# seorim0/DNN-based-Speech-Enhancement-in-the-frequency-domain

Measured on AMD Instinct MI355X. Metric: train utts/sec (3s@16kHz) DCCRN, higher is better.
Workload: dtype bf16; 1 GPU; DCCRN mask C, SI-SNR, fwd+bwd+Adam, B=32/GPU x 3s@16kHz clips (BASELINE configs[1]); global_batch=32, parallelism=dp1, bn=per-rank statistics, collective=none

## Files before the change

dnn-based-speech-enhancement-in-the-frequency-domain_amd/csrc/dev_common.h:

```cpp
#pragma once
#include <hip/hip_runtime.h>
#include "sefd_desc.h"

namespace sefd {

typedef __attribute__((ext_vector_type(4))) float f32x4;
typedef __attribute__((ext_vector_type(16))) float f32x16;
typedef __attribute__((ext_vector_type(8))) __bf16 bf16x8;

struct bf16_t { uint16_t v; };

struct ArenaBases { char* p[A_COUNT]; int* status; int* dstatus; };
__device__ __forceinline__ void set_status(int* host_word, int* dev_word) {
  if (host_word) __hip_atomic_store(host_word, 1, __ATOMIC_RELAXED, __HIP_MEMORY_SCOPE_SYSTEM);
  if (dev_word) __hip_atomic_store(dev_word, 1, __ATOMIC_RELAXED, __HIP_MEMORY_SCOPE_AGENT);
}

__host__ __device__ __forceinline__ char* rp(const ArenaBases& ab, const Ptr& q) { return ab.p[q.arena] + q.off; }

__device__ __forceinline__ uint32_t pack_bf16x2(float lo, float hi) {
  uint32_t r;
  asm("v_cvt_pk_bf16_f32 %0, %1, %2" : "=v"(r) : "v"(lo), "v"(hi));
  return r;
}
// ... 92 lines not shown
__device__ __forceinline__ float tanhf_(float x) { return 1.f - 2.f * __builtin_amdgcn_rcpf(__expf(2.f * x) + 1.f); }

__device__ __forceinline__ uint32_t mix32(uint32_t a, uint32_t b, uint32_t c) {
  uint32_t x = a * 0x9E3779B1u ^ (b + 0x7F4A7C15u) * 0x85EBCA77u ^ (c + 0x632BE5ABu) * 0xC2B2AE3Du;
  x ^= x >> 16; x *= 0x7FEB352Du; x ^= x >> 15; x *= 0x846CA68Bu; x ^= x >> 16;
  return x;
}
__device__ __forceinline__ float drop_scale(uint32_t seed0, uint32_t seed1, int layer, float keep, int64_t i) {
  if (keep >= 1.f) return 1.f;
  const uint32_t r = mix32(seed0 + (uint32_t)layer * 0x51ED27u, seed1 ^ (uint32_t)(i >> 32), (uint32_t)i);
  return ((r >> 8) * (1.f / 16777216.f)) < keep ? 1.f / keep : 0.f;
}

struct BnbCol { float mean, invstd, gamma, beta; };
__device__ __forceinline__ BnbCol bnb_col(const RunGemm& d, const ArenaBases& ab, int n) {
  BnbCol c{0.f, 0.f, 0.f, 0.f};
  if (n < d.N) {
    const float* mi = reinterpret_cast<const float*>(rp(ab, d.bnb_mi));
    c.mean = mi[n]; c.invstd = mi[d.N + n];
    c.gamma = reinterpret_cast<const float*>(rp(ab, d.bnb_gamma))[n];
    c.beta = reinterpret_cast<const float*>(rp(ab, d.bnb_beta))[n];
  }
  return c;
}
__device__ __forceinline__ void bnb_accum(const BnbCol& c, float slope, float dz, float yf, float& s0, float& s1, float& s2) {
  const float xh = (yf - c.mean) * c.invstd;
  const float bn = c.gamma * xh + c.beta;
  const float dbn = bn > 0.f ? dz : slope * dz;
  s0 += dbn;
  s1 += dbn * xh;
  s2 += bn > 0.f ? 0.f : bn * dz;
}

struct StreamKey {
  int dev; hipStream_t st;
  bool operator==(const StreamKey& o) const { return dev == o.dev && st == o.st; }
};
struct StreamKeyHash { size_t operator()(const StreamKey& k) const { return (size_t)(uintptr_t)k.st * 31u + (size_t)k.dev; } };
inline StreamKey stream_key(hipStream_t st) { int dev = 0; (void)hipGetDevice(&dev); return StreamKey{dev, st}; }

void launch_rungemm(const RunGemm& d, const ArenaBases& ab, hipStream_t st);
void launch_wgrad(const RunGemm& d, const ArenaBases& ab, hipStream_t st);
bool launch_cgemm256(const RunGemm& d, const ArenaBases& ab, hipStream_t st);
bool launch_enc0_fwd(const RunGemm& d, const ArenaBases& ab, hipStream_t st);
bool launch_enc0_wgrad(const RunGemm& d, const ArenaBases& ab, hipStream_t st);
bool launch_rundirect(const RunGemm& d, const ArenaBases& ab, hipStream_t st);
bool rundirect_takes(const RunGemm& d);
bool launch_rungemm_persist(const RunGemm& d, const ArenaBases& ab, hipStream_t st);
int rungemm_persist_grid(const RunGemm& d);
bool launch_thin_mask(const RunGemm& d, const ArenaBases& ab, hipStream_t st);
int thin_mask_grid(const RunGemm& d);
bool launch_thin_stage(const RunGemm& d, const ArenaBases& ab, hipStream_t st);
int thin_stage_grid(const RunGemm& d);
enum RunFamily : int { kFamNone = 0, kFamEnc0 = 1, kFamCgemm256 = 2, kFamDirect = 3, kFamTiled = 4, kFamPersist = 5, kFamThinMask = 6, kFamThinStage = 7 };
int rungemm_family(const RunGemm& d);
enum WgradFamily : int { kWgFamNone = 0, kWgFamEnc0 = 1, kWgFamEnc0Fused = 2, kWgFamRank = 3, kWgFamWide256 = 4, kWgFamWide256Ones = 5, kWgFamWide128 = 6,
                         kWgFamDma128 = 7, kWgFamDma64 = 8, kWgFamDma32 = 9, kWgFamBf16_128 = 10, kWgFamBf16_64 = 11, kWgFamF32 = 12, kWgFamThin = 13 };
int wgrad_family(const RunGemm& d);
bool launch_thin_wgrad(const RunGemm& d, const ArenaBases& ab, hipStream_t st);
bool thin_wgrad_takes(const RunGemm& d);
void launch_misc(const Op& op, const ArenaBases& ab, hipStream_t st);
void launch_stft_fft(const StftFft& d, const ArenaBases& ab, hipStream_t st);
void launch_istft_fft(const IstftFft& d, const ArenaBases& ab, hipStream_t st);
void launch_ifft_ola(const IfftOla& d, const ArenaBases& ab, hipStream_t st);
void launch_specconv(const SpecConv& d, const ArenaBases& ab, hipStream_t st);
void launch_ola_fold(const Ola& d, const ArenaBases& ab, hipStream_t st);
void launch_specout_adj(const SpecOut& d, const ArenaBases& ab, hipStream_t st);
void launch_nchw_cl(const NchwCl& d, const ArenaBases& ab, hipStream_t st);
void launch_fsn(const Op& op, const ArenaBases& ab, hipStream_t st);
void launch_bn(const Op& op, const ArenaBases& ab, hipStream_t st);
void launch_cbn(const Op& op, const ArenaBases& ab, hipStream_t st);
void launch_lstm_bf16(const LstmRec& d, const ArenaBases& ab, hipStream_t st, bool fwd);
inline int lstm_rev_groups(const LstmRec& d) { return d.rev_mask & ((1 << (d.G < 4 ? d.G : 4)) - 1); }
void launch_lstm_cluster(const LstmRec& d, const ArenaBases& ab, hipStream_t st, bool fwd);
void launch_lstm_rows(const LstmRec& d, const ArenaBases& ab, hipStream_t st, bool fwd);
bool launch_lstm_rows_pair(const LstmRec& d0, const LstmRec& d1, const ArenaBases& ab, hipStream_t st);

}
```

dnn-based-speech-enhancement-in-the-frequency-domain_amd/csrc/rungemm.hip:

```cpp
#include <hip/hip_runtime.h>
#include <cstdlib>
#include "sefd_desc.h"
#include "tuning.h"
#include "dev_common.h"

namespace sefd {

template <typename TA>
struct RowInfo {
  int64_t base0, base1;
  int32_t u, fo;
  bool valid;
};

template <typename TA>
__device__ __forceinline__ uint4 load_a_chunk(const RunGemm& d, const TA* x0, const TA* x1, const Seg& sg,
                                              int64_t base0, int64_t base1, int u, int fo, bool rvalid, int j0) {
  constexpr int VEC = 16 / sizeof(TA);
  uint4 z = make_uint4(0, 0, 0, 0);
  if (!rvalid) return z;
  if (sg.src < 0) {
    if (j0 == 0) {
      if (sizeof(TA) == 4) z.x = 0x3f800000u; else z.x = 0x3f80u;
    }
// ... 1106 lines not shown
}

static bool launch_wgrad_rank(const RunGemm& d, const ArenaBases& ab, hipStream_t st) {
  if (!(d.flags & kRunRank) || !wgrad_rank_form(d)) return false;
  const dim3 grid((unsigned)d.nsplit);
  if (d.N <= 2) hipLaunchKernelGGL((wgrad_rank_kernel<2>), grid, dim3(256), 0, st, d, ab);
  else hipLaunchKernelGGL((wgrad_rank_kernel<4>), grid, dim3(256), 0, st, d, ab);
  return true;
}

template <typename TA, int BN>
static void launch_rungemm_dma(const RunGemm& d, const ArenaBases& ab, hipStream_t st, int grid) {
  if (d.flags & kRunBnBwd) { hipLaunchKernelGGL((rungemm_kernel<TA, BN, true, 2, kBM, 4, false, true>), dim3(grid), dim3(256), 0, st, d, ab); return; }
  hipLaunchKernelGGL((rungemm_kernel<TA, BN, true, 2>), dim3(grid), dim3(256), 0, st, d, ab);
}

template <typename TA>
static void launch_rungemm_t(const RunGemm& d, const ArenaBases& ab, hipStream_t st) {
  const int bn = bn_of(d.N);
  const int nm = (d.M + kBM - 1) / kBM;
  const int grid = nm * (d.Npad / bn);
  if constexpr (sizeof(TA) == 2) {
    if (launch_rungemm_persist(d, ab, st)) return;
  }
  if (d.flags & kRunAligned) {
    if (bn == 128) launch_rungemm_dma<TA, 128>(d, ab, st, grid);
    else if (bn == 64) launch_rungemm_dma<TA, 64>(d, ab, st, grid);
    else launch_rungemm_dma<TA, 32>(d, ab, st, grid);
    return;
  }
  if (d.flags & kRunBnBwd) {
    if (bn == 128) hipLaunchKernelGGL((rungemm_kernel<TA, 128, false, 2, kBM, 4, false, true>), dim3(grid), dim3(256), 0, st, d, ab);
    else if (bn == 64) hipLaunchKernelGGL((rungemm_kernel<TA, 64, false, 2, kBM, 4, false, true>), dim3(grid), dim3(256), 0, st, d, ab);
    else hipLaunchKernelGGL((rungemm_kernel<TA, 32, false, 2, kBM, 4, false, true>), dim3(grid), dim3(256), 0, st, d, ab);
    return;
  }
  if (bn == 128) hipLaunchKernelGGL((rungemm_kernel<TA, 128, false>), dim3(grid), dim3(256), 0, st, d, ab);
  else if (bn == 64) hipLaunchKernelGGL((rungemm_kernel<TA, 64, false>), dim3(grid), dim3(256), 0, st, d, ab);
  else hipLaunchKernelGGL((rungemm_kernel<TA, 32, false>), dim3(grid), dim3(256), 0, st, d, ab);
}

__global__ void refuse_launch_kernel(int* host_word, int* dev_word) { set_status(host_word, dev_word); }

static void refuse_launch(const ArenaBases& ab, hipStream_t st) {
  hipLaunchKernelGGL(refuse_launch_kernel, dim3(1), dim3(1), 0, st, ab.status, ab.dstatus);
}

void launch_rungemm(const RunGemm& d, const ArenaBases& ab, hipStream_t st) {
  if (launch_enc0_fwd(d, ab, st)) return;
  if (d.flags & (kRunEnc0 | kRunDyFromBn)) { refuse_launch(ab, st); return; }
  if (launch_cgemm256(d, ab, st)) return;
  if (launch_thin_mask(d, ab, st)) return;
  if (launch_thin_stage(d, ab, st)) return;
  if (launch_rundirect(d, ab, st)) return;
  if (d.xdt == DT_BF16) launch_rungemm_t<bf16_t>(d, ab, st);
  else launch_rungemm_t<float>(d, ab, st);
}

int rungemm_family(const RunGemm& d) {
  if ((d.flags & kRunEnc0) && enc0_accepts(d, false)) return kFamEnc0;
  if (d.flags & (kRunEnc0 | kRunDyFromBn)) return kFamNone;
  if (d.flags & kRunWTile32) return kFamCgemm256;
  if (thin_mask_grid(d) > 0) return kFamThinMask;
  if (thin_stage_grid(d) > 0) return kFamThinStage;
  if (rundirect_takes(d)) return kFamDirect;
  if (d.xdt == DT_BF16 && rungemm_persist_grid(d) > 0) return kFamPersist;
  return kFamTiled;
}

static void launch_wgrad_wide(const RunGemm& d, const ArenaBases& ab, hipStream_t st) {
  if (d.flags & kRunOnesMfma) {
    dim3 grid1(((d.Npad + 255) / 256) * ((d.ldw - 64 + 255) / 256) * d.nsplit);
    hipLaunchKernelGGL((wgrad_bf16_dma_kernel<256, 4, 256, 512, true, true>), grid1, dim3(512), 0, st, d, ab);
    return;
  }
  dim3 grid(((d.Npad + 255) / 256) * ((d.ldw + 255) / 256) * d.nsplit);
  hipLaunchKernelGGL((wgrad_bf16_dma_kernel<256, 4, 256, 512, true>), grid, dim3(512), 0, st, d, ab);
}

static void launch_wgrad_wide128(const RunGemm& d, const ArenaBases& ab, hipStream_t st) {
  dim3 grid(((d.Npad + 127) / 128) * ((d.ldw + 511) / 512) * d.nsplit);
  hipLaunchKernelGGL((wgrad_bf16_dma_kernel<128, 2, 512, 512>), grid, dim3(512), 0, st, d, ab);
}

template <int TN>
static void launch_wgrad_dma(const RunGemm& d, const ArenaBases& ab, hipStream_t st) {
  dim3 grid(((d.Npad + TN - 1) / TN) * ((d.ldw + kWgTK - 1) / kWgTK) * d.nsplit);
  hipLaunchKernelGGL((wgrad_bf16_dma_kernel<TN, 3>), grid, dim3(256), 0, st, d, ab);
}

void launch_wgrad(const RunGemm& d0, const ArenaBases& ab, hipStream_t st) {
  if (launch_enc0_wgrad(d0, ab, st)) return;
  if (d0.flags & (kRunEnc0 | kRunDyFromBn)) { refuse_launch(ab, st); return; }
  if (launch_wgrad_rank(d0, ab, st)) return;
  RunGemm d = d0;
#ifdef SEFD_TUNING
  if (tune_int("WG_DBG", 0) & 8) d.flags |= 1 << 30;
#endif
  if (d.xdt == DT_BF16 && (d.flags & kRunAligned)) {
    if (d.flags & kRunWgWide) { if (d.Npad % 256 == 0) launch_wgrad_wide(d, ab, st); else launch_wgrad_wide128(d, ab, st); return; }
    if (launch_thin_wgrad(d0, ab, st)) return;
    switch (wgrad_tn(d.xdt, d.N, d.Npad)) {
      case 128: launch_wgrad_dma<128>(d, ab, st); break;
      case 64: launch_wgrad_dma<64>(d, ab, st); break;
      default: launch_wgrad_dma<32>(d, ab, st); break;
    }
    return;
  }
  if (d.xdt == DT_BF16) {
    if (d.Npad >= 128) {
      dim3 grid(((d.Npad + 127) / 128) * ((d.ldw + kWgTK - 1) / kWgTK) * d.nsplit);
      hipLaunchKernelGGL((wgrad_bf16_kernel<128>), grid, dim3(256), 0, st, d, ab);
    } else {
      dim3 grid(((d.Npad + 63) / 64) * ((d.ldw + kWgTK - 1) / kWgTK) * d.nsplit);
      hipLaunchKernelGGL((wgrad_bf16_kernel<64>), grid, dim3(256), 0, st, d, ab);
    }
    return;
// ... 24 lines not shown
```

dnn-based-speech-enhancement-in-the-frequency-domain_amd/csrc/thin_stage.hip:

```cpp
#include <hip/hip_runtime.h>
#include <cstdlib>
#include "sefd_desc.h"
#include "tuning.h"
#include "dev_common.h"

namespace sefd {

namespace {

constexpr int kStageFo = 64;
constexpr int64_t kThinStageMinRows = 262144;

__device__ __forceinline__ void settle(f32x4& a, f32x4& b) { asm volatile("s_nop 7\n\ts_nop 7" : "+v"(a), "+v"(b)); }
__device__ __forceinline__ void settle(f32x4& a, f32x4& b, f32x4& c, f32x4& e) { asm volatile("s_nop 7\n\ts_nop 7" : "+v"(a), "+v"(b), "+v"(c), "+v"(e)); }

template <int CTRL>
__device__ __forceinline__ float dpp_f(float x) {
  return __builtin_bit_cast(float, __builtin_amdgcn_update_dpp(0, __builtin_bit_cast(int, x), CTRL, 0xF, 0xF, true));
}
__device__ __forceinline__ void chain32(float a, float b, float& t1, float& t2) {
  constexpr int SHR1 = 0x111, SHR5 = 0x115, SHL11 = 0x10B, SHL4 = 0x104;
  float s = 0.f + a, r = __builtin_fmaf(a, a, 0.f);
#pragma unroll
  for (int k = 0; k < 3; ++k) { s = dpp_f<SHR1>(s) + a; r = __builtin_fmaf(a, a, dpp_f<SHR1>(r)); }
  s = dpp_f<SHR5>(s) + a; r = __builtin_fmaf(a, a, dpp_f<SHR5>(r));
#pragma unroll
  for (int k = 0; k < 3; ++k) { s = dpp_f<SHR1>(s) + a; r = __builtin_fmaf(a, a, dpp_f<SHR1>(r)); }
  s = dpp_f<SHL11>(s) + b; r = __builtin_fmaf(b, b, dpp_f<SHL11>(r));
#pragma unroll
  for (int k = 0; k < 3; ++k) { s = dpp_f<SHR1>(s) + b; r = __builtin_fmaf(b, b, dpp_f<SHR1>(r)); }
  s = dpp_f<SHR5>(s) + b; r = __builtin_fmaf(b, b, dpp_f<SHR5>(r));
#pragma unroll
  for (int k = 0; k < 3; ++k) { s = dpp_f<SHR1>(s) + b; r = __builtin_fmaf(b, b, dpp_f<SHR1>(r)); }
  t1 = s + dpp_f<SHL4>(s);
  t2 = r + dpp_f<SHL4>(r);
}
__device__ __forceinline__ void chain32(const f32x4& a, const f32x4& b, f32x4& t1, f32x4& t2) {
#pragma unroll
  for (int e = 0; e < 4; ++e) { float x, y; chain32(a[e], b[e], x, y); t1[e] = x; t2[e] = y; }
}

template <int C, int NSRC>
struct StageGeom {
  static constexpr int CH = NSRC * C / 8;
  static constexpr int PB = CH * 16;
  static constexpr int SLOT = (kStageFo + 2) * PB;
  static constexpr int CPT = C / 8;
  static constexpr int HS = C / 32;
  static constexpr int NSEG = 2 * NSRC;
  static constexpr int KS = NSEG * 3 * HS;
  static constexpr int NIT = kStageFo * CH / 256;
  static constexpr int RPL = PB >= 256 ? 1 : 256 / PB;
  static constexpr int NT = C / 16;
  static constexpr int NPG = 4 / NT;
  static constexpr int NB = kStageFo / 16 / NPG;
  static constexpr int RED = NPG > 1 ? 2 * 4 * 2 * 4 * 16 : 0;
  static_assert((C == 64 || C == 32) && (NSRC == 1 || NSRC == 2) && NIT >= 1 && NB % 2 == 0 && NT * NPG == 4 && (NPG == 1 || NB == 2), "instantiated forms");
  __host__ __device__ static constexpr int swz(int pos) { return (pos / RPL) & (CH - 1); }
};

}

template <int C, int NSRC>
// ... 118 lines not shown
        float* prow = part + (int64_t)(g >> 1) * 2 * d.Npad + 16 * ct + 4 * q;
        if constexpr (G::NPG == 1) {
          if (fr == 0) { s1 = f32x4{0.f, 0.f, 0.f, 0.f}; s2 = s1; }
#pragma unroll
          for (int j = 0; j < NB / 2; ++j) {
            f32x4 t1, t2;
            chain32(acc[2 * j], acc[2 * j + 1], t1, t2);
            s1 += t1; s2 += t2;
          }
          if (rowend && li == 11) {
            *reinterpret_cast<f32x4*>(prow) = s1;
            *reinterpret_cast<f32x4*>(prow + d.Npad) = s2;
          }
        } else {
          f32x4* red = reinterpret_cast<f32x4*>(smem + 3 * SLOT);
          f32x4 t1, t2;
          chain32(acc[0], acc[1], t1, t2);
          if (li == 11) { red[((fr * 4 + wid) * 2 + 0) * 4 + q] = t1; red[((fr * 4 + wid) * 2 + 1) * 4 + q] = t2; }
          if (rowend) {
            lds_barrier();
            if (pg == 0 && li == 11) {
              f32x4 a1 = {0.f, 0.f, 0.f, 0.f}, a2 = a1;
              for (int f = 0; f <= fr; ++f)
#pragma unroll
                for (int h = 0; h < G::NPG; ++h) { a1 += red[((f * 4 + ct + h * NT) * 2 + 0) * 4 + q]; a2 += red[((f * 4 + ct + h * NT) * 2 + 1) * 4 + q]; }
              *reinterpret_cast<f32x4*>(prow) = a1;
              *reinterpret_cast<f32x4*>(prow + d.Npad) = a2;
            }
          }
        }
      }

      uint16_t* yrow = y + (int64_t)cb * d.y_bstride + (int64_t)cu * d.y_tstride + d.y_off + 16 * ct + (odd ? 4 * (q - 1) : 4 * q);
#pragma unroll
      for (int j = 0; j < NB / 2; ++j) {
        const f32x4 &A = acc[2 * j], &B = acc[2 * j + 1];
        const uint32_t X0 = pack_bf16x2(A[0], A[1]), X1 = pack_bf16x2(A[2], A[3]);
        const uint32_t Y0 = pack_bf16x2(B[0], B[1]), Y1 = pack_bf16x2(B[2], B[3]);
        const uint32_t r0 = (uint32_t)__shfl_xor((int)(odd ? X0 : Y0), 16), r1 = (uint32_t)__shfl_xor((int)(odd ? X1 : Y1), 16);
        const uint4 o4 = odd ? make_uint4(r0, r1, Y0, Y1) : make_uint4(X0, X1, r0, r1);
        const int f = pg * 16 * NB + 16 * (2 * j + (odd ? 1 : 0)) + li;
        *reinterpret_cast<uint4*>(yrow + (int64_t)f * d.y_fstride) = o4;
      }
      --left;
    }
    cb = nb; cu = nu;
    if (++nu == Tout) { nu = ustart; ++nb; }
    const int t = sp; sp = sc; sc = sn; sn = t;
  }
}

namespace {

template <int C, int NCP>
struct StrideGeom {
  static constexpr int CPT = C / 8;
  static constexpr int PB = CPT * 16;
  static constexpr int PLANE = (kStageFo + 2) * PB;
  static constexpr int SLOT = 2 * PLANE;
  static constexpr int KS = 2 * 5 * C / 32;
  static constexpr int NIT = 2 * kStageFo * CPT / 256;
  static constexpr int RPL = 256 / PB;
  static constexpr int NPH = NCP == 4 ? 1 : 2;
  static constexpr int NB = 4 / NPH;
  static constexpr int RED = NPH > 1 ? 2 * 4 * 2 * 8 * 16 : 0;
  static_assert((C == 32 || C == 16) && (NCP == 1 || NCP == 2 || NCP == 4) && NIT >= 1 && (2 * 5 * C) % 32 == 0, "instantiated forms");
  __host__ __device__ static constexpr int swz(int row) { return (row / RPL) & (CPT - 1); }
};

}

template <int C, int NCP>
__global__ __launch_bounds__(256) __attribute__((amdgpu_waves_per_eu(NCP == 4 ? 2 : 3))) void thin_stage_st_kernel(const RunGemm d, const ArenaBases ab) {
  using G = StrideGeom<C, NCP>;
  constexpr int CPT = G::CPT, PB = G::PB, PLANE = G::PLANE, SLOT = G::SLOT, KS = G::KS, NIT = G::NIT, NB = G::NB;
  __shared__ __attribute__((aligned(16))) char smem[3 * SLOT + G::RED];
  const int tid = threadIdx.x, lane = tid & 63, wid = __builtin_amdgcn_readfirstlane(tid >> 6);
  const int li = lane & 15, q = lane >> 4;
  const int cp = wid % NCP, ph = wid / NCP;
  const bool active = ph < G::NPH;

  const int Tout = d.Tout, Tin = d.Tin[0];
  const int nframes = (int)(d.M / kStageFo), nrows = (nframes + 1) >> 1;
  const int g0 = 2 * (int)((int64_t)blockIdx.x * nrows / gridDim.x);
  int g1 = 2 * (int)((int64_t)(blockIdx.x + 1) * nrows / gridDim.x);
  if (g1 > nframes) g1 = nframes;
  if (g0 >= g1) return;

  const uint16_t* x0 = reinterpret_cast<const uint16_t*>(rp(ab, d.x[0]));
  const uint16_t* zp = reinterpret_cast<const uint16_t*>(rp(ab, d.zero));
  const uint16_t* w = reinterpret_cast<const uint16_t*>(rp(ab, d.w));
  uint16_t* y = reinterpret_cast<uint16_t*>(rp(ab, d.y));
  uint16_t* y2 = d.n2 > 0 ? reinterpret_cast<uint16_t*>(rp(ab, d.y2)) - d.n2 : y;
  const int n2 = d.n2 > 0 ? d.n2 : 0x7fffffff;
  float* part = d.stats.arena >= 0 ? reinterpret_cast<float*>(rp(ab, d.stats)) : nullptr;

  const int hi = d.seg[0].dt > d.seg[1].dt ? d.seg[0].dt : d.seg[1].dt;
  const bool lo0 = d.seg[0].dt != hi, lo1 = d.seg[1].dt != hi;
  const int ustart = (hi == 0 && Tout - 1 >= Tin) ? 0 : -1;

  uint4 wreg[2][KS];
  int koff[KS];
  bool klo[KS];
#pragma unroll
  for (int ks = 0; ks < KS; ++ks) {
    int run, tap, cc;
    if constexpr (CPT == 4) { run = ks / 5; tap = ks % 5; cc = q; }
    else { const int cid = 4 * ks + q; run = cid / (5 * CPT); tap = (cid - run * 5 * CPT) / CPT; cc = cid % CPT; }
    klo[ks] = run ? lo1 : lo0;
    const int ko = run ? d.seg[1].koff : d.seg[0].koff;
#pragma unroll
    for (int h = 0; h < 2; ++h) {
      const int n = 32 * cp + 8 * (li >> 2) + 4 * h + (li & 3);
      wreg[h][ks] = *reinterpret_cast<const uint4*>(w + (int64_t)n * d.ldw + ko + tap * C + cc * 8);
    }
    const int row = ph * 16 * NB + li + (tap >> 1);
    koff[ks] = (tap & 1) * PLANE + row * PB + ((cc ^ G::swz(row)) << 4);
  }
  f32x4 bias4[2] = {{0.f, 0.f, 0.f, 0.f}, {0.f, 0.f, 0.f, 0.f}};
  if (d.bias.arena >= 0) {
    const float* bp = reinterpret_cast<const float*>(rp(ab, d.bias));
#pragma unroll
    for (int h = 0; h < 2; ++h)
#pragma unroll
      for (int e = 0; e < 4; ++e) bias4[h][e] = bp[32 * cp + 8 * q + 4 * h + e];
  }

  int eoff[NIT], edst[NIT];
#pragma unroll
  for (int it = 0; it < NIT; ++it) {
    const int L = it * 256 + tid, plane = L / (kStageFo * CPT), within = L % (kStageFo * CPT), row = 1 + within / CPT, c = (within % CPT) ^ G::swz(row);
    eoff[it] = (2 * (row - 1) + plane) * C + c * 8;
    const int L0 = it * 256 + wid * 64;
    edst[it] = (L0 / (kStageFo * CPT)) * PLANE + PB + (L0 % (kStageFo * CPT)) * 16;
  }
  const uint32_t lbase = lds_addr(smem);
  const int64_t bs0 = d.bstride[0];
  const int ts0 = d.tstride[0], ba0 = d.base[0];
  auto issue_frame = [&](int b, int t, int slot) {
    const bool valid = t >= 0 && t < Tin;
    const uint16_t* f0 = x0 + (int64_t)b * bs0 + ba0 + (int64_t)t * ts0;
#pragma unroll
    for (int it = 0; it < NIT; ++it) dma16(valid ? f0 + eoff[it] : zp, lbase + slot + edst[it]);
  };
  if (tid < 12 * CPT) {
    const int r = tid / CPT, slot = r / 4, plane = (r >> 1) & 1, last = r & 1;
    *reinterpret_cast<uint4*>(smem + slot * SLOT + plane * PLANE + (last ? (kStageFo + 1) * PB : 0) + (tid % CPT) * 16) = make_uint4(0, 0, 0, 0);
  }

  int cb = g0 / Tout, cu = g0 - cb * Tout;
  int sp = 0, sc = SLOT, sn = 2 * SLOT;
  issue_frame(cb, cu + hi - 1, sp);
  issue_frame(cb, cu + hi, sc);
  int nb = cb, nu = cu + 1;
  if (nu == Tout) { nu = ustart; ++nb; }
  f32x4 s1[2] = {{0.f, 0.f, 0.f, 0.f}, {0.f, 0.f, 0.f, 0.f}}, s2[2] = {{0.f, 0.f, 0.f, 0.f}, {0.f, 0.f, 0.f, 0.f}};
  int left = g1 - g0;
  __builtin_amdgcn_s_waitcnt(0x0F70);

  while (left > 0) {
    wait_vm<0>();
    lds_barrier();
    const bool out = cu >= 0;
    if (left - (out ? 1 : 0) > 0) issue_frame(nb, nu + hi, sn);
    if (out) {
      const int g = g1 - left;
      f32x4 acc[2][NB];
#pragma unroll
      for (int blk = 0; blk < NB; ++blk) acc[0][blk] = acc[1][blk] = f32x4{0.f, 0.f, 0.f, 0.f};
      if (active) {
      auto frag = [&](int ks, uint4 (&b)[NB]) {
        const int off = (klo[ks] ? sp : sc) + koff[ks];
#pragma unroll
        for (int blk = 0; blk < NB; ++blk) b[blk] = *reinterpret_cast<const uint4*>(smem + off + blk * 16 * PB);
      };
      uint4 bf[2][NB];
      frag(0, bf[0]);
#pragma unroll
      for (int ks = 0; ks < KS; ++ks) {
        if (ks + 1 < KS) frag(ks + 1, bf[(ks + 1) & 1]);
        __builtin_amdgcn_sched_barrier(0);
#pragma unroll
        for (int blk = 0; blk < NB; ++blk) {
          const bf16x8 bfr = __builtin_bit_cast(bf16x8, bf[ks & 1][blk]);
          acc[0][blk] = __builtin_amdgcn_mfma_f32_16x16x32_bf16(__builtin_bit_cast(bf16x8, wreg[0][ks]), bfr, acc[0][blk], 0, 0, 0);
          acc[1][blk] = __builtin_amdgcn_mfma_f32_16x16x32_bf16(__builtin_bit_cast(bf16x8, wreg[1][ks]), bfr, acc[1][blk], 0, 0, 0);
        }
        __builtin_amdgcn_sched_barrier(0);
      }
#pragma unroll
      for (int blk = 0; blk < NB; ++blk) { acc[0][blk] += bias4[0]; acc[1][blk] += bias4[1]; }
      }

      if (part) {
        const int fr = (g - g0) & 1;
        const bool rowend = fr != 0 || left == 1;
        float* prow = part + (int64_t)(g >> 1) * 2 * d.Npad + 32 * cp + 8 * q;
        if constexpr (G::NPH == 1) {
          if (fr == 0) { s1[0] = s1[1] = s2[0] = s2[1] = f32x4{0.f, 0.f, 0.f, 0.f}; }
#pragma unroll
          for (int j = 0; j < NB / 2; ++j)
#pragma unroll
            for (int h = 0; h < 2; ++h) {
              f32x4 t1, t2;
              chain32(acc[h][2 * j], acc[h][2 * j + 1], t1, t2);
              s1[h] += t1; s2[h] += t2;
            }
          if (rowend && li == 11) {
#pragma unroll
            for (int h = 0; h < 2; ++h) {
              *reinterpret_cast<f32x4*>(prow + 4 * h) = s1[h];
              *reinterpret_cast<f32x4*>(prow + d.Npad + 4 * h) = s2[h];
            }
          }
        } else {
          f32x4* red = reinterpret_cast<f32x4*>(smem + 3 * SLOT);
          if (active) {
#pragma unroll
            for (int h = 0; h < 2; ++h) {
              f32x4 t1, t2;
              chain32(acc[h][0], acc[h][1], t1, t2);
              if (li == 11) { red[((fr * 4 + wid) * 2 + 0) * 8 + q * 2 + h] = t1; red[((fr * 4 + wid) * 2 + 1) * 8 + q * 2 + h] = t2; }
            }
          }
          if (rowend) {
            lds_barrier();
            if (ph == 0 && li == 11) {
#pragma unroll
              for (int h = 0; h < 2; ++h) {
                f32x4 a1 = {0.f, 0.f, 0.f, 0.f}, a2 = a1;
                for (int f = 0; f <= fr; ++f)
#pragma unroll
                  for (int hh = 0; hh < G::NPH; ++hh) {
                    a1 += red[((f * 4 + cp + hh * NCP) * 2 + 0) * 8 + q * 2 + h];
                    a2 += red[((f * 4 + cp + hh * NCP) * 2 + 1) * 8 + q * 2 + h];
                  }
                *reinterpret_cast<f32x4*>(prow + 4 * h) = a1;
                *reinterpret_cast<f32x4*>(prow + d.Npad + 4 * h) = a2;
              }
            }
          }
        }
      }

      const int n0 = 32 * cp + 8 * q;
      uint16_t* yrow = (n0 >= n2 ? y2 : y) + (int64_t)cb * d.y_bstride + (int64_t)cu * d.y_tstride + d.y_off + n0;
#pragma unroll
      for (int blk = 0; blk < NB; ++blk) {
        const uint4 o4 = make_uint4(pack_bf16x2(acc[0][blk][0], acc[0][blk][1]), pack_bf16x2(acc[0][blk][2], acc[0][blk][3]),
                                    pack_bf16x2(acc[1][blk][0], acc[1][blk][1]), pack_bf16x2(acc[1][blk][2], acc[1][blk][3]));
        const int f = 16 * (ph * NB + blk) + li;
        if (active) *reinterpret_cast<uint4*>(yrow + (int64_t)f * d.y_fstride) = o4;
      }
      --left;
    }
    cb = nb; cu = nu;
    if (++nu == Tout) { nu = ustart; ++nb; }
    const int t = sp; sp = sc; sc = sn; sn = t;
  }
}

namespace {

bool stage_common(const RunGemm& d) {
  if (d.xdt != DT_BF16 || d.ydt != DT_BF16 || !(d.flags & kRunAligned) || !(d.flags & kRunYAligned)) return false;
  if (d.flags & (kRunAccum | kRunRelu | kRunBnBwd | kRunWTile32 | kRunEnc0 | kRunDyFromBn | kRunRank)) return false;
  if (d.zero.arena < 0 || d.M <= 0 || d.Tout <= 0 || d.Fo != kStageFo || (int64_t)d.M % ((int64_t)d.Tout * d.Fo) != 0 || d.x[0].arena < 0) return false;
  if (d.y_fstride % 8 != 0 || d.y_off % 8 != 0 || d.y_tstride % 8 != 0 || d.y_bstride % 8 != 0 || d.ldw % 8 != 0) return false;
  if (d.n2 != 0 && (d.n2 < 0 || d.n2 % 8 != 0 || d.n2 >= d.N || d.y2.arena < 0)) return false;
  if (d.stats.arena >= 0 && (d.Npad != d.N || d.n2 != 0 || d.stats.off % 16 != 0)) return false;
  return d.Tin[0] > 0 && d.tstride[0] % 8 == 0 && d.base[0] % 8 == 0 && d.bstride[0] % 8 == 0;
}

bool stage_runs(const RunGemm& d, int nsrc, int off, int len) {
  if (d.nseg != 2 * nsrc) return false;
  const int hi = d.seg[0].dt > d.seg[1].dt ? d.seg[0].dt : d.seg[1].dt;
  if (hi != 0 && hi != 1) return false;
  for (int sg = 0; sg < 2 * nsrc; ++sg) {
    const Seg& s = d.seg[sg];
    if (s.src != (sg >> 1) || (s.dt != hi && s.dt != hi - 1) || s.off != off || s.len != len || s.koff % 8 != 0 || s.koff < 0 || s.koff + s.len > d.ldw) return false;
    if ((sg & 1) && s.dt == d.seg[sg - 1].dt) return false;
  }
  return true;
}

int stage_pm_form(const RunGemm& d) {
  if (!stage_common(d) || d.n2 != 0) return 0;
  const int nsrc = d.x[1].arena >= 0 ? 2 : 1, C = d.fstride[0];
  if ((C != 64 && C != 32) || d.N != C) return 0;
  for (int s = 0; s < nsrc; ++s)
    if (d.fstride[s] != C || d.rowlen[s] != d.Fo * C || d.Tin[s] != d.Tin[0] || d.tstride[s] % 8 != 0 || d.base[s] % 8 != 0 || d.bstride[s] % 8 != 0) return 0;
  return stage_runs(d, nsrc, -C, 3 * C) ? C + 256 * nsrc : 0;
}

int stage_st_form(const RunGemm& d) {
  if (!stage_common(d) || d.x[1].arena >= 0 || d.fstride[0] % 2 != 0 || d.N % 32 != 0) return 0;
  const int C = d.fstride[0] / 2, ncp = d.N / 32;
  if (!((C == 32 && (ncp == 2 || ncp == 4)) || (C == 16 && (ncp == 1 || ncp == 2)))) return 0;
  if (d.rowlen[0] != 2 * d.Fo * C) return 0;
  if (d.stats.arena < 0 && d.n2 == 0) return 0;
  return stage_runs(d, 1, -2 * C, 5 * C) ? C + 256 * ncp : 0;
}

int stage_form(const RunGemm& d) {
  const int pm = stage_pm_form(d);
  if (pm) return pm;
  const int st = stage_st_form(d);
  return st ? st + 65536 : 0;
}

int stage_cus() {
  static const int ncu = [] {
    int dev = 0, n = 0;
    if (hipGetDevice(&dev) != hipSuccess || hipDeviceGetAttribute(&n, hipDeviceAttributeMultiprocessorCount, dev) != hipSuccess || n <= 0) {
      (void)hipGetLastError();
      return 256;
    }
    return n;
  }();
  return ncu;
}

template <typename K>
int stage_wgs_per_cu(K kern, int fallback) {
  int q = 0;
  if (hipOccupancyMaxActiveBlocksPerMultiprocessor(&q, reinterpret_cast<const void*>(kern), 256, 0) != hipSuccess || q <= 0) {
    (void)hipGetLastError();
    return fallback;
  }
  return q;
}

int stage_resident(int form) {
  switch (form) {
    case 64 + 512: { static const int n = stage_wgs_per_cu(&thin_stage_pm_kernel<64, 2>, 2); return n; }
    case 64 + 256: { static const int n = stage_wgs_per_cu(&thin_stage_pm_kernel<64, 1>, 2); return n; }
    case 32 + 512: { static const int n = stage_wgs_per_cu(&thin_stage_pm_kernel<32, 2>, 4); return n; }
    case 32 + 256: { static const int n = stage_wgs_per_cu(&thin_stage_pm_kernel<32, 1>, 4); return n; }
    case 65536 + 32 + 512: { static const int n = stage_wgs_per_cu(&thin_stage_st_kernel<32, 2>, 3); return n; }
    case 65536 + 32 + 1024: { static const int n = stage_wgs_per_cu(&thin_stage_st_kernel<32, 4>, 2); return n; }
    case 65536 + 16 + 256: { static const int n = stage_wgs_per_cu(&thin_stage_st_kernel<16, 1>, 4); return n; }
    default: { static const int n = stage_wgs_per_cu(&thin_stage_st_kernel<16, 2>, 4); return n; }
  }
}

}

int thin_stage_grid(const RunGemm& d) {
  const int mode = (int)tune_int("THIN_STAGE", 1);
  if (mode <= 0) return 0;
  const int form = stage_form(d);
  if (!form) return 0;
  if (mode != 2 && d.M < kThinStageMinRows) return 0;
  const int64_t units = (d.M / kStageFo + 1) / 2;
  int64_t grid = (int64_t)stage_resident(form) * stage_cus();
  const int64_t forced = tune_int("THIN_STAGE_GRID", 0);
  if (forced > 0) grid = forced;
  if (grid > units) grid = units;
  return (int)(grid < 1 ? 1 : grid);
}

bool launch_thin_stage(const RunGemm& d, const ArenaBases& ab, hipStream_t st) {
  const int grid = thin_stage_grid(d);
  if (grid <= 0) return false;
  switch (stage_form(d)) {
    case 64 + 512: hipLaunchKernelGGL((thin_stage_pm_kernel<64, 2>), dim3(grid), dim3(256), 0, st, d, ab); break;
    case 64 + 256: hipLaunchKernelGGL((thin_stage_pm_kernel<64, 1>), dim3(grid), dim3(256), 0, st, d, ab); break;
    case 32 + 512: hipLaunchKernelGGL((thin_stage_pm_kernel<32, 2>), dim3(grid), dim3(256), 0, st, d, ab); break;
    case 32 + 256: hipLaunchKernelGGL((thin_stage_pm_kernel<32, 1>), dim3(grid), dim3(256), 0, st, d, ab); break;
    case 65536 + 32 + 512: hipLaunchKernelGGL((thin_stage_st_kernel<32, 2>), dim3(grid), dim3(256), 0, st, d, ab); break;
    case 65536 + 32 + 1024: hipLaunchKernelGGL((thin_stage_st_kernel<32, 4>), dim3(grid), dim3(256), 0, st, d, ab); break;
    case 65536 + 16 + 256: hipLaunchKernelGGL((thin_stage_st_kernel<16, 1>), dim3(grid), dim3(256), 0, st, d, ab); break;
    default: hipLaunchKernelGGL((thin_stage_st_kernel<16, 2>), dim3(grid), dim3(256), 0, st, d, ab); break;
  }
  return true;
}

}
```

dnn-based-speech-enhancement-in-the-frequency-domain_amd/plan.py:

```python
import ctypes as C
from collections import OrderedDict

import numpy as np
import torch

from . import _lib

ARENA_WS, ARENA_PARAM, ARENA_GRAD, ARENA_STATE, ARENA_CONST, ARENA_IO, ARENA_COUNT = 0, 1, 2, 3, 4, 5, 6
PHASE_FWD, PHASE_BWD = 0, 1
RUN_FAMILY_NONE, RUN_FAMILY_ENC0, RUN_FAMILY_CGEMM256, RUN_FAMILY_DIRECT, RUN_FAMILY_TILED, RUN_FAMILY_PERSIST, RUN_FAMILY_THIN_MASK, RUN_FAMILY_THIN_STAGE = range(8)
(WG_FAMILY_NONE, WG_FAMILY_ENC0, WG_FAMILY_ENC0_FUSED, WG_FAMILY_RANK, WG_FAMILY_WIDE256, WG_FAMILY_WIDE256_ONES, WG_FAMILY_WIDE128,
 WG_FAMILY_DMA128, WG_FAMILY_DMA64, WG_FAMILY_DMA32, WG_FAMILY_BF16_128, WG_FAMILY_BF16_64, WG_FAMILY_F32, WG_FAMILY_THIN) = range(14)
WG_FAMILY_NAMES = ("none", "first layer", "first layer fused", "rank-N", "256 x 256", "256 x 256 ones MFMA", "128 x 512", "aligned 128", "aligned 64",
                   "aligned 32", "unaligned bf16 128", "unaligned bf16 64", "fp32")
WG_FAMILY_MORE_NAMES = {WG_FAMILY_THIN: "frame-staged thin"}


def wg_family_name(family):
    return WG_FAMILY_MORE_NAMES[family] if family in WG_FAMILY_MORE_NAMES else WG_FAMILY_NAMES[family]
RUN_WAVE_ONLY = 1
MASK_MODES = {"E": 0, "C": 1, "R": 2, "Direct(None make)": 4}
DTYPES = {"fp32": 0, "float32": 0, "bf16": 1, "bfloat16": 1}


CONV_KINDS = {"ComplexConv2d": 0, "ComplexConvTranspose2d": 1, "RealConv2d": 2, "RealConvTranspose2d": 3}
FSN_NORMS = {"offline_laplace_norm": 0, "cumulative_laplace_norm": 1, "offline_gaussian_norm": 2, "cumulative_layer_norm": 3}


class Plan:
    def __init__(self, B, L, kernel_num=(32, 64, 128, 256, 256, 256), rnn_layers=2, rnn_units=256, win_len=400,
                 win_inc=100, fft_len=512, masking_mode="E", lstm="complex", skip_type=True, act_dtype="fp32",
                 kernel_size=5, training=True, model="DCCRN", fsn=None, bn_world=1, grad_buckets=1, use_cbn=False, win_type="hanning",
                 cbn_sync=False, seq=None, feature_type="complex", conv=None, cbn=None, clstm=None):
        self.lib = _lib.lib()
        if masking_mode not in MASK_MODES:
            raise NotImplementedError(f"masking_mode {masking_mode!r} is not on the HIP path yet")
        cfg = _lib.ModelConfig()
        cfg.model = {"DCCRN": 0, "CRN": 1, "STFT": 2, "FullSubNet": 3, "TorchSTFT": 4, "TorchISTFT": 5, "SequenceModel": 6, "ConvSTFT": 7,
                     "ConviSTFT": 8, "ConvLayer": 9, "ComplexBatchNorm": 10, "ComplexLSTM": 11, "TorchSTFTAdj": 12, "TorchISTFTAdj": 13}[model]
        cfg.B, cfg.L = int(B), int(L)
        if model == "FullSubNet":
            f = dict(sb_num_neighbors=15, fb_num_neighbors=0, look_ahead=2, fb_hidden=512, sb_hidden=384, fb_act="ReLU",
                     sb_act=None, keep=0.2, sequence_model="LSTM", norm_type="offline_laplace_norm")
            f.update(fsn or {})
            acts = {None: 0, "None": 0, "ReLU": 1, "Tanh": 2, "ReLU6": 3}
            kernel_num = (f["sb_num_neighbors"], f["fb_num_neighbors"], f["look_ahead"], f["fb_hidden"], f["sb_hidden"],
                          acts[f["fb_act"]], acts[f["sb_act"]], int(round(f["keep"] * 1000)),
                          {"LSTM": 0, "GRU": 1}[f["sequence_model"]], FSN_NORMS[f["norm_type"]])
        if model == "SequenceModel":
            s = dict(input_size=257, output_size=257, hidden_size=512, num_layers=2, bidirectional=False, sequence_model="LSTM", keep=0.2)
            s.update(seq or {})
            if s["sequence_model"] not in ("LSTM", "GRU"):
                raise NotImplementedError(f"Not implemented {s['sequence_model']}")
            kernel_num = (s["input_size"], s["output_size"], s["hidden_size"], s["num_layers"], 1 if s["bidirectional"] else 0,
                          {"LSTM": 0, "GRU": 1}[s["sequence_model"]], int(round(s["keep"] * 1000)))
            self.seq = s
        if model in ("ConvSTFT", "ConviSTFT"):
            kernel_num = (0 if feature_type == "complex" else 1,)
        if model == "ConvLayer":
            v = dict(kind="ComplexConv2d", in_channels=2, out_channels=2, kernel_size=(1, 1), stride_f=1, padding=(0, 0), causal=True, output_padding_f=0, F=1)
            v.update(conv or {})
            kernel_num = (CONV_KINDS[v["kind"]], v["in_channels"], v["out_channels"], v["kernel_size"][0], v["kernel_size"][1], v["stride_f"],
                          v["padding"][0], v["padding"][1], 1 if v["causal"] else 0, v["output_padding_f"], v["F"])
# ... 211 lines not shown
```

Baseline: 3288 utt/s.

## Add frame-staged strided kernel path for 64-channel, 32-frequency conv layers

Extends the frame-staged strided conv kernel to take the frame width as a template parameter and instantiates a 64-channel, Fo=32 form. That form packs four frames per stats row and reduces BN statistics through an extra LDS tile. The form is dispatched ahead of the direct and tiled GEMM paths for matching encoder layers. The aim is to replace the generic GEMM path for that layer shape with a fused, LDS-staged kernel. It adds LDS use and a new statistics reduction scheme that could lower occupancy or hide layout bugs.

Result: faster. 3335 utt/s, median of 6 (+1.4%).

```diff
diff --git a/dnn-based-speech-enhancement-in-the-frequency-domain_amd/csrc/dev_common.h b/dnn-based-speech-enhancement-in-the-frequency-domain_amd/csrc/dev_common.h
--- a/dnn-based-speech-enhancement-in-the-frequency-domain_amd/csrc/dev_common.h
+++ b/dnn-based-speech-enhancement-in-the-frequency-domain_amd/csrc/dev_common.h
@@ -168,7 +168,9 @@
 int thin_mask_grid(const RunGemm& d);
 bool launch_thin_stage(const RunGemm& d, const ArenaBases& ab, hipStream_t st);
 int thin_stage_grid(const RunGemm& d);
-enum RunFamily : int { kFamNone = 0, kFamEnc0 = 1, kFamCgemm256 = 2, kFamDirect = 3, kFamTiled = 4, kFamPersist = 5, kFamThinMask = 6, kFamThinStage = 7 };
+bool launch_thin_stage64(const RunGemm& d, const ArenaBases& ab, hipStream_t st);
+int thin_stage64_grid(const RunGemm& d);
+enum RunFamily : int { kFamNone = 0, kFamEnc0 = 1, kFamCgemm256 = 2, kFamDirect = 3, kFamTiled = 4, kFamPersist = 5, kFamThinMask = 6, kFamThinStage = 7, kFamThinStage64 = 8 };
 int rungemm_family(const RunGemm& d);
 enum WgradFamily : int { kWgFamNone = 0, kWgFamEnc0 = 1, kWgFamEnc0Fused = 2, kWgFamRank = 3, kWgFamWide256 = 4, kWgFamWide256Ones = 5, kWgFamWide128 = 6,
                          kWgFamDma128 = 7, kWgFamDma64 = 8, kWgFamDma32 = 9, kWgFamBf16_128 = 10, kWgFamBf16_64 = 11, kWgFamF32 = 12, kWgFamThin = 13 };
diff --git a/dnn-based-speech-enhancement-in-the-frequency-domain_amd/csrc/rungemm.hip b/dnn-based-speech-enhancement-in-the-frequency-domain_amd/csrc/rungemm.hip
--- a/dnn-based-speech-enhancement-in-the-frequency-domain_amd/csrc/rungemm.hip
+++ b/dnn-based-speech-enhancement-in-the-frequency-domain_amd/csrc/rungemm.hip
@@ -1182,6 +1182,7 @@
   if (launch_cgemm256(d, ab, st)) return;
   if (launch_thin_mask(d, ab, st)) return;
   if (launch_thin_stage(d, ab, st)) return;
+  if (launch_thin_stage64(d, ab, st)) return;
   if (launch_rundirect(d, ab, st)) return;
   if (d.xdt == DT_BF16) launch_rungemm_t<bf16_t>(d, ab, st);
   else launch_rungemm_t<float>(d, ab, st);
@@ -1193,6 +1194,7 @@
   if (d.flags & kRunWTile32) return kFamCgemm256;
   if (thin_mask_grid(d) > 0) return kFamThinMask;
   if (thin_stage_grid(d) > 0) return kFamThinStage;
+  if (thin_stage64_grid(d) > 0) return kFamThinStage64;
   if (rundirect_takes(d)) return kFamDirect;
   if (d.xdt == DT_BF16 && rungemm_persist_grid(d) > 0) return kFamPersist;
   return kFamTiled;
diff --git a/dnn-based-speech-enhancement-in-the-frequency-domain_amd/csrc/thin_stage.hip b/dnn-based-speech-enhancement-in-the-frequency-domain_amd/csrc/thin_stage.hip
--- a/dnn-based-speech-enhancement-in-the-frequency-domain_amd/csrc/thin_stage.hip
+++ b/dnn-based-speech-enhancement-in-the-frequency-domain_amd/csrc/thin_stage.hip
@@ -9,6 +9,7 @@
 namespace {
 
 constexpr int kStageFo = 64;
+constexpr int kStage64Fo = 32;
 constexpr int64_t kThinStageMinRows = 262144;
 
 __device__ __forceinline__ void settle(f32x4& a, f32x4& b) { asm volatile("s_nop 7\n\ts_nop 7" : "+v"(a), "+v"(b)); }
@@ -233,38 +234,43 @@
 
 namespace {
 
-template <int C, int NCP>
+template <int C, int NCP, int FO>
 struct StrideGeom {
   static constexpr int CPT = C / 8;
   static constexpr int PB = CPT * 16;
-  static constexpr int PLANE = (kStageFo + 2) * PB;
+  static constexpr int PLANE = (FO + 2) * PB;
   static constexpr int SLOT = 2 * PLANE;
   static constexpr int KS = 2 * 5 * C / 32;
-  static constexpr int NIT = 2 * kStageFo * CPT / 256;
+  static constexpr int NIT = 2 * FO * CPT / 256;
   static constexpr int RPL = 256 / PB;
+  static constexpr int FPR = 128 / FO;
   static constexpr int NPH = NCP == 4 ? 1 : 2;
-  static constexpr int NB = 4 / NPH;
+  static constexpr int NB = FO / 16 / NPH;
   static constexpr int RED = NPH > 1 ? 2 * 4 * 2 * 8 * 16 : 0;
-  static_assert((C == 32 || C == 16) && (NCP == 1 || NCP == 2 || NCP == 4) && NIT >= 1 && (2 * 5 * C) % 32 == 0, "instantiated forms");
+  static constexpr bool TILE = FO == 32;
+  static constexpr int TP = 32 * NCP + 4;
+  static constexpr int TILEB = TILE ? 32 * TP * 4 : 0;
+  static_assert((!TILE || FPR == 4) && ((FO == 64 && (C == 32 || C == 16) && (NCP == 1 || NCP == 2 || NCP == 4)) || (FO == 32 && C == 64 && NCP == 4)) && NIT >= 1 &&
+                (2 * 5 * C) % 32 == 0 && NB % 2 == 0 && (!TILE || (NPH == 1 && NB == 2)), "instantiated forms");
   __host__ __device__ static constexpr int swz(int row) { return (row / RPL) & (CPT - 1); }
 };
 
 }
 
-template <int C, int NCP>
+template <int C, int NCP, int FO = kStageFo>
 __global__ __launch_bounds__(256) __attribute__((amdgpu_waves_per_eu(NCP == 4 ? 2 : 3))) void thin_stage_st_kernel(const RunGemm d, const ArenaBases ab) {
-  using G = StrideGeom<C, NCP>;
-  constexpr int CPT = G::CPT, PB = G::PB, PLANE = G::PLANE, SLOT = G::SLOT, KS = G::KS, NIT = G::NIT, NB = G::NB;
-  __shared__ __attribute__((aligned(16))) char smem[3 * SLOT + G::RED];
+  using G = StrideGeom<C, NCP, FO>;
+  constexpr int CPT = G::CPT, PB = G::PB, PLANE = G::PLANE, SLOT = G::SLOT, KS = G::KS, NIT = G::NIT, NB = G::NB, FPR = G::FPR;
+  __shared__ __attribute__((aligned(16))) char smem[3 * SLOT + G::RED + G::TILEB];
   const int tid = threadIdx.x, lane = tid & 63, wid = __builtin_amdgcn_readfirstlane(tid >> 6);
   const int li = lane & 15, q = lane >> 4;
   const int cp = wid % NCP, ph = wid / NCP;
   const bool active = ph < G::NPH;
 
   const int Tout = d.Tout, Tin = d.Tin[0];
-  const int nframes = (int)(d.M / kStageFo), nrows = (nframes + 1) >> 1;
-  const int g0 = 2 * (int)((int64_t)blockIdx.x * nrows / gridDim.x);
-  int g1 = 2 * (int)((int64_t)(blockIdx.x + 1) * nrows / gridDim.x);
+  const int nframes = (int)(d.M / FO), nrows = (nframes + FPR - 1) / FPR;
+  const int g0 = FPR * (int)((int64_t)blockIdx.x * nrows / gridDim.x);
+  int g1 = FPR * (int)((int64_t)(blockIdx.x + 1) * nrows / gridDim.x);
   if (g1 > nframes) g1 = nframes;
   if (g0 >= g1) return;
 
@@ -310,10 +316,10 @@
   int eoff[NIT], edst[NIT];
 #pragma unroll
   for (int it = 0; it < NIT; ++it) {
-    const int L = it * 256 + tid, plane = L / (kStageFo * CPT), within = L % (kStageFo * CPT), row = 1 + within / CPT, c = (within % CPT) ^ G::swz(row);
+    const int L = it * 256 + tid, plane = L / (FO * CPT), within = L % (FO * CPT), row = 1 + within / CPT, c = (within % CPT) ^ G::swz(row);
     eoff[it] = (2 * (row - 1) + plane) * C + c * 8;
     const int L0 = it * 256 + wid * 64;
-    edst[it] = (L0 / (kStageFo * CPT)) * PLANE + PB + (L0 % (kStageFo * CPT)) * 16;
+    edst[it] = (L0 / (FO * CPT)) * PLANE + PB + (L0 % (FO * CPT)) * 16;
   }
   const uint32_t lbase = lds_addr(smem);
   const int64_t bs0 = d.bstride[0];
@@ -326,7 +332,7 @@
   };
   if (tid < 12 * CPT) {
     const int r = tid / CPT, slot = r / 4, plane = (r >> 1) & 1, last = r & 1;
-    *reinterpret_cast<uint4*>(smem + slot * SLOT + plane * PLANE + (last ? (kStageFo + 1) * PB : 0) + (tid % CPT) * 16) = make_uint4(0, 0, 0, 0);
+    *reinterpret_cast<uint4*>(smem + slot * SLOT + plane * PLANE + (last ? (FO + 1) * PB : 0) + (tid % CPT) * 16) = make_uint4(0, 0, 0, 0);
   }
 
   int cb = g0 / Tout, cu = g0 - cb * Tout;
@@ -373,7 +379,39 @@
       for (int blk = 0; blk < NB; ++blk) { acc[0][blk] += bias4[0]; acc[1][blk] += bias4[1]; }
       }
 
-      if (part) {
+      if constexpr (G::TILE) {
+        if (part) {
+          float* tile = reinterpret_cast<float*>(smem + 3 * SLOT + G::RED);
+#pragma unroll
+          for (int blk = 0; blk < NB; ++blk)
+#pragma unroll
+            for (int h = 0; h < 2; ++h) *reinterpret_cast<f32x4*>(tile + (16 * blk + li) * G::TP + 32 * cp + 8 * q + 4 * h) = acc[h][blk];
+          lds_barrier();
+          const int fr = (g - g0) % FPR, col = tid >> 1, hh = tid & 1;
+          if (fr == 0) { s1[0][0] = 0.f; s2[0][0] = 0.f; }
+          if ((fr & 1) == 0) { s1[0][1] = 0.f; s2[0][1] = 0.f; }
+          float s = s1[0][1], r = s2[0][1];
+#pragma unroll
+          for (int k = 0; k < 4; ++k)
+#pragma unroll
+            for (int rr = 0; rr < 4; ++rr) {
+              const float v = tile[(4 * hh + 8 * k + rr) * G::TP + col];
+              s = s + v;
+              r = __builtin_fmaf(v, v, r);
+            }
+          s1[0][1] = s; s2[0][1] = r;
+          const bool rowend = fr == FPR - 1 || left == 1;
+          if ((fr & 1) != 0 || rowend) {
+            s1[0][0] += s + dpp_f<0xB1>(s);
+            s2[0][0] += r + dpp_f<0xB1>(r);
+          }
+          if (rowend && hh == 0) {
+            float* prow = part + (int64_t)(g / FPR) * 2 * d.Npad + col;
+            prow[0] = s1[0][0];
+            prow[d.Npad] = s2[0][0];
+          }
+        }
+      } else if (part) {
         const int fr = (g - g0) & 1;
         const bool rowend = fr != 0 || left == 1;
         float* prow = part + (int64_t)(g >> 1) * 2 * d.Npad + 32 * cp + 8 * q;
@@ -443,10 +481,10 @@
 
 namespace {
 
-bool stage_common(const RunGemm& d) {
+bool stage_common(const RunGemm& d, int fo = kStageFo) {
   if (d.xdt != DT_BF16 || d.ydt != DT_BF16 || !(d.flags & kRunAligned) || !(d.flags & kRunYAligned)) return false;
   if (d.flags & (kRunAccum | kRunRelu | kRunBnBwd | kRunWTile32 | kRunEnc0 | kRunDyFromBn | kRunRank)) return false;
-  if (d.zero.arena < 0 || d.M <= 0 || d.Tout <= 0 || d.Fo != kStageFo || (int64_t)d.M % ((int64_t)d.Tout * d.Fo) != 0 || d.x[0].arena < 0) return false;
+  if (d.zero.arena < 0 || d.M <= 0 || d.Tout <= 0 || d.Fo != fo || (int64_t)d.M % ((int64_t)d.Tout * d.Fo) != 0 || d.x[0].arena < 0) return false;
   if (d.y_fstride % 8 != 0 || d.y_off % 8 != 0 || d.y_tstride % 8 != 0 || d.y_bstride % 8 != 0 || d.ldw % 8 != 0) return false;
   if (d.n2 != 0 && (d.n2 < 0 || d.n2 % 8 != 0 || d.n2 >= d.N || d.y2.arena < 0)) return false;
   if (d.stats.arena >= 0 && (d.Npad != d.N || d.n2 != 0 || d.stats.off % 16 != 0)) return false;
@@ -488,6 +526,14 @@
   if (pm) return pm;
   const int st = stage_st_form(d);
   return st ? st + 65536 : 0;
+}
+
+bool stage64_form(const RunGemm& d) {
+  if (!stage_common(d, kStage64Fo) || (d.flags & ~(kRunAligned | kRunYAligned)) != 0 || d.x[1].arena >= 0) return false;
+  constexpr int C = 64;
+  if (d.fstride[0] != 2 * C || d.N != 128 || d.Npad != 128 || d.rowlen[0] != 2 * d.Fo * C) return false;
+  if (d.stats.arena < 0 && d.bias.arena >= 0) return false;
+  return stage_runs(d, 1, -2 * C, 5 * C);
 }
 
 int stage_cus() {
@@ -525,6 +571,28 @@
   }
 }
 
+int stage64_resident() { static const int n = stage_wgs_per_cu(&thin_stage_st_kernel<64, 4, kStage64Fo>, 2); return n; }
+
+}
+
+int thin_stage64_grid(const RunGemm& d) {
+  const int mode = (int)tune_int("THIN_STAGE64", 1);
+  if (mode <= 0 || !stage64_form(d)) return 0;
+  if (mode != 2 && d.M < kThinStageMinRows) return 0;
+  constexpr int fpr = 128 / kStage64Fo;
+  const int64_t units = (d.M / kStage64Fo + fpr - 1) / fpr;
+  int64_t grid = (int64_t)stage64_resident() * stage_cus();
+  const int64_t forced = tune_int("THIN_STAGE64_GRID", 0);
+  if (forced > 0) grid = forced;
+  if (grid > units) grid = units;
+  return (int)(grid < 1 ? 1 : grid);
+}
+
+bool launch_thin_stage64(const RunGemm& d, const ArenaBases& ab, hipStream_t st) {
+  const int grid = thin_stage64_grid(d);
+  if (grid <= 0) return false;
+  hipLaunchKernelGGL((thin_stage_st_kernel<64, 4, kStage64Fo>), dim3(grid), dim3(256), 0, st, d, ab);
+  return true;
 }
 
 int thin_stage_grid(const RunGemm& d) {
diff --git a/dnn-based-speech-enhancement-in-the-frequency-domain_amd/plan.py b/dnn-based-speech-enhancement-in-the-frequency-domain_amd/plan.py
--- a/dnn-based-speech-enhancement-in-the-frequency-domain_amd/plan.py
+++ b/dnn-based-speech-enhancement-in-the-frequency-domain_amd/plan.py
@@ -9,6 +9,8 @@
 ARENA_WS, ARENA_PARAM, ARENA_GRAD, ARENA_STATE, ARENA_CONST, ARENA_IO, ARENA_COUNT = 0, 1, 2, 3, 4, 5, 6
 PHASE_FWD, PHASE_BWD = 0, 1
 RUN_FAMILY_NONE, RUN_FAMILY_ENC0, RUN_FAMILY_CGEMM256, RUN_FAMILY_DIRECT, RUN_FAMILY_TILED, RUN_FAMILY_PERSIST, RUN_FAMILY_THIN_MASK, RUN_FAMILY_THIN_STAGE = range(8)
+RUNGEMM_FAMILY_THIN_STAGE64 = 8
+RUNGEMM_FAMILY_MORE_NAMES = {RUNGEMM_FAMILY_THIN_STAGE64: "frame-staged 64-channel strided"}
 (WG_FAMILY_NONE, WG_FAMILY_ENC0, WG_FAMILY_ENC0_FUSED, WG_FAMILY_RANK, WG_FAMILY_WIDE256, WG_FAMILY_WIDE256_ONES, WG_FAMILY_WIDE128,
  WG_FAMILY_DMA128, WG_FAMILY_DMA64, WG_FAMILY_DMA32, WG_FAMILY_BF16_128, WG_FAMILY_BF16_64, WG_FAMILY_F32, WG_FAMILY_THIN) = range(14)
 WG_FAMILY_NAMES = ("none", "first layer", "first layer fused", "rank-N", "256 x 256", "256 x 256 ones MFMA", "128 x 512", "aligned 128", "aligned 64",
```
